# finmath/finmath-lib-cuda-extensions

Measured on AMD Instinct MI355X. Metric: Monte-Carlo path-ops/sec (fused RandomVariable stream), higher is better.
Workload: dtype f32

## Files before the change

finmath-lib-cuda-extensions_amd/host/hip_backend.hpp:

```cpp
#pragma once
#include <cstdlib>
#include <cstring>
#include <memory>
#include "lmm.hpp"

namespace fmhost {

class BrownianMotionFromMersenneRandomNumbersHip final : public BrownianMotion {
public:
    BrownianMotionFromMersenneRandomNumbersHip(TimeDiscretization td, int numberOfFactors, int64_t numberOfPaths, int seed, int64_t pathOffset = 0)
        : td_(std::move(td)), factors_(numberOfFactors), paths_(numberOfPaths), offset_(pathOffset), seed_(seed) {}
    RV getBrownianIncrement(int timeIndex, int factor) const override {
        std::call_once(generated_, [this] { generate(); });
        return inc_.at((size_t)timeIndex * factors_ + factor);
    }
    const TimeDiscretization& getTimeDiscretization() const override { return td_; }
    int getNumberOfFactors() const override { return factors_; }
    int64_t getNumberOfPaths() const override { return paths_; }
    int getSeed() const { return seed_; }
    RV getRandomVariableForConstant(double value) const override { return RandomVariableHip::of(-std::numeric_limits<double>::infinity(), value); }
private:
    void generate() const {
        const int steps = td_.getNumberOfTimeSteps();
        std::vector<double> dt((size_t)steps);
        for (int i = 0; i < steps; ++i) dt[(size_t)i] = td_.getTimeStep(i);
        std::vector<fmhip_vec> h((size_t)steps * factors_);
        check(fmhip_bm_generate_mersenne_device(seed_, steps, factors_, paths_, offset_, dt.data(), h.data()));
        inc_.reserve(h.size());
        for (int i = 0; i < steps; ++i)
            for (int f = 0; f < factors_; ++f)
                inc_.push_back(RandomVariableHip::of(td_.getTime(i + 1), DeviceVector(h[(size_t)i * factors_ + f]), paths_));
    }
    TimeDiscretization td_;
    int factors_;
    int64_t paths_, offset_;
    int seed_;
    mutable std::vector<RV> inc_;
    mutable std::once_flag generated_;
};

inline lmm::Backend makeHipBackend(const RandomVariableFactory* factory, const BrownianMotion* brownianMotion, int chunk = 0, int stepsPerLaunch = 0, int jacobianBatch = 0) {
    lmm::Backend be;
    be.factory = factory;
    be.brownianMotion = brownianMotion;
    if (!(std::getenv("FMHIP_LMM_FLUSH") && std::getenv("FMHIP_LMM_FLUSH")[0] == '0'))
        be.flush = [] { check(fmhip_flush()); };
    if (!(std::getenv("FMHIP_LMM_HOLD") && std::getenv("FMHIP_LMM_HOLD")[0] == '0'))
        be.hold = [](bool h) { check(fmhip_fusion_hold(h ? 1 : 0, nullptr)); };
    if (chunk > 0) be.chunk = chunk;
    if (stepsPerLaunch > 0) be.stepsPerLaunch = stepsPerLaunch;
    be.jacobianBatch = jacobianBatch > 0 ? jacobianBatch : 8;
    if (!(std::getenv("FMHIP_LMM_CLONE") && std::getenv("FMHIP_LMM_CLONE")[0] == '0')) {
        auto handleOf = [](const RV& x) {
            auto p = dynamic_cast<const RandomVariableHip*>(x.get());
            if (!p || p->isDeterministic()) throw std::runtime_error("graph replication over a value that is not a device vector");
            return p->deviceVector().handle();
        };
        be.clone = [handleOf](const std::vector<RV>& roots, const std::vector<RV>& leafFrom, const std::vector<std::vector<RV>>& leafTo,
                              const std::vector<std::vector<double>>* scalars) {
            const int nRoots = (int)roots.size(), nMap = (int)leafFrom.size(), nCopies = (int)leafTo.size();
            std::vector<fmhip_vec> r, lf, lt, out((size_t)nRoots * nCopies);
            for (const RV& x : roots) r.push_back(handleOf(x));
            for (const RV& x : leafFrom) lf.push_back(handleOf(x));
            for (const auto& row : leafTo) { if ((int)row.size() != nMap) throw std::runtime_error("graph replication: ragged operand map"); for (const RV& x : row) lt.push_back(handleOf(x)); }
            std::vector<double> sc;
            int nScalars = 0;
            if (scalars) { nScalars = (int)(*scalars)[0].size(); for (const auto& row : *scalars) { if ((int)row.size() != nScalars) throw std::runtime_error("graph replication: ragged scalar lists"); sc.insert(sc.end(), row.begin(), row.end()); } }
            check(fmhip_graph_clone(r.data(), nRoots, nCopies, lf.data(), lt.data(), nMap, scalars ? sc.data() : nullptr, nScalars, out.data()));
            std::vector<std::vector<RV>> copies((size_t)nCopies);
            for (int c = 0; c < nCopies; ++c)
                for (int k = 0; k < nRoots; ++k)
                    copies[(size_t)c].push_back(RandomVariableHip::of(roots[(size_t)k]->getFiltrationTime(), DeviceVector(out[(size_t)c * nRoots + k]), roots[(size_t)k]->size()));
            return copies;
        };
        be.recordedScalars = [handleOf](const std::vector<RV>& roots) {
            std::vector<fmhip_vec> r;
            for (const RV& x : roots) r.push_back(handleOf(x));
            int n = 0;
            check(fmhip_graph_scalars(r.data(), (int)r.size(), nullptr, 0, &n));
            std::vector<double> sc((size_t)n);
            check(fmhip_graph_scalars(r.data(), (int)r.size(), sc.data(), n, &n));
            return sc;
        };
    }
    if (!(std::getenv("FMHIP_LMM_DISCARD") && std::getenv("FMHIP_LMM_DISCARD")[0] == '0'))
        be.valuesNotNeeded = [](const std::vector<RV>& v) {
            std::vector<fmhip_vec> h;
            for (const RV& x : v) { auto p = dynamic_cast<const RandomVariableHip*>(x.get()); if (p && !p->isDeterministic()) h.push_back(p->deviceVector().handle()); }
            if (!h.empty()) check(fmhip_vec_give_up_values(h.data(), (int)h.size()));
        };
    be.launches = [] { fmhip_engine_stats_t s; check(fmhip_engine_stats(&s)); return (long long)s.kernel_launches; };
    be.averages = [](const std::vector<RV>& v) { return getAverages(v); };
    if (!(std::getenv("FMHIP_LMM_ASYNC") && std::getenv("FMHIP_LMM_ASYNC")[0] == '0'))
        be.expectationsRunPending = true;
    if (!(std::getenv("FMHIP_LMM_ASYNC") && std::getenv("FMHIP_LMM_ASYNC")[0] == '0'))
        be.averagesAsync = [](const std::vector<RV>& v) -> std::function<std::vector<double>()> {
            std::vector<fmhip_vec> h;
            int64_t n = 0;
            for (const RV& x : v) {
                auto p = dynamic_cast<const RandomVariableHip*>(x.get());
                if (!p || p->isDeterministic()) { const std::vector<double> now = getAverages(v); return [now] { return now; }; }
                h.push_back(p->deviceVector().handle()); n = p->size();
            }
            const int count = (int)h.size();
            fmhip_ticket ticket = 0;
            check(fmhip_reduce_moments_batch_begin(h.data(), count, nullptr, &ticket));
            struct Owner { fmhip_ticket t = 0; int count = 0; bool ended = false;
                           Owner() = default; Owner(const Owner&) = delete; Owner& operator=(const Owner&) = delete;
                           ~Owner() { if (!ended && t) { std::vector<fmhip_moments> drop((size_t)count); (void)fmhip_reduce_moments_batch_end(t, drop.data(), count); } } };
            auto owner = std::make_shared<Owner>();
            owner->t = ticket; owner->count = count;
            return [owner, count, n] {
                std::vector<fmhip_moments> m((size_t)count);
                owner->ended = true;
                check(fmhip_reduce_moments_batch_end(owner->t, m.data(), count));
                std::vector<double> out((size_t)count);
                for (int k = 0; k < count; ++k) out[(size_t)k] = m[(size_t)k].sum / (double)n;
                return out;
            };
        };
    return be;
}

}
```

finmath-lib-cuda-extensions_amd/host/lmm.hpp:

```cpp
#pragma once
#include <algorithm>
#include <chrono>
#include <cmath>
#include <cstdio>
#include <atomic>
#include <thread>
#include <cstdlib>
#include <functional>
#include <string>
#include <vector>

#include "random_variable.hpp"

namespace fmhost { namespace lmm {


inline const std::vector<double>& atmNormalVolatilities() {
    static const std::vector<double> v = {
        0.00151, 0.00169, 0.0021, 0.00248, 0.00291, 0.00329, 0.00365, 0.004, 0.00437, 0.00466, 0.00527, 0.00571,
        0.00604, 0.00625, 0.0016, 0.00174, 0.00217, 0.00264, 0.00314, 0.00355, 0.00398, 0.00433, 0.00469,
        0.00493, 0.00569, 0.00607, 0.00627, 0.00645, 0.00182, 0.00204, 0.00238, 0.00286, 0.00339, 0.00384,
        0.00424, 0.00456, 0.00488, 0.0052, 0.0059, 0.00623, 0.0064, 0.00654, 0.00205, 0.00235, 0.00272, 0.0032,
        0.00368, 0.00406, 0.00447, 0.00484, 0.00515, 0.00544, 0.00602, 0.00629, 0.0064, 0.00646, 0.00279,
        0.00319, 0.0036, 0.00396, 0.00436, 0.00469, 0.00503, 0.0053, 0.00557, 0.00582, 0.00616, 0.00628,
        0.00638, 0.00641, 0.00379, 0.00406, 0.00439, 0.00472, 0.00504, 0.00532, 0.0056, 0.00582, 0.00602,
        0.00617, 0.0063, 0.00636, 0.00638, 0.00639, 0.00471, 0.00489, 0.00511, 0.00539, 0.00563, 0.00583, 0.006,
        0.00618, 0.0063, 0.00644, 0.00641, 0.00638, 0.00635, 0.00634, 0.00544, 0.00557, 0.00572, 0.00591,
        0.00604, 0.00617, 0.0063, 0.00641, 0.00651, 0.00661, 0.00645, 0.00634, 0.00627, 0.00624, 0.00625,
        0.00632, 0.00638, 0.00644, 0.0065, 0.00655, 0.00661, 0.00667, 0.00672, 0.00673, 0.00634, 0.00614,
        0.00599, 0.00593, 0.00664, 0.00671, 0.00675, 0.00676, 0.00676, 0.00675, 0.00676, 0.00674, 0.00672,
        0.00669, 0.00616, 0.00586, 0.00569, 0.00558, 0.00647, 0.00651, 0.00651, 0.00651, 0.00652, 0.00649,
        0.00645, 0.0064, 0.00637, 0.00631, 0.00576, 0.00534, 0.00512, 0.00495, 0.00615, 0.0062, 0.00618,
        0.00613, 0.0061, 0.00607, 0.00602, 0.00596, 0.00591, 0.00586, 0.00536, 0.00491, 0.00469, 0.0045,
        0.00578, 0.00583, 0.00579, 0.00574, 0.00567, 0.00562, 0.00556, 0.00549, 0.00545, 0.00538, 0.00493,
        0.00453, 0.00435, 0.0042, 0.00542, 0.00547, 0.00539, 0.00532, 0.00522, 0.00516, 0.0051, 0.00504, 0.005,
        0.00495, 0.00454, 0.00418, 0.00404, 0.00394 };
    return v;
}
inline const std::vector<double>& atmExpiryYears() { static const std::vector<double> v = { 1.0 / 12, 0.25, 0.5, 1, 2, 3, 4, 5, 7, 10, 15, 20, 25, 30 }; return v; }
inline const std::vector<double>& atmTenorYears()  { static const std::vector<double> v = { 1, 2, 3, 4, 5, 6, 7, 8, 9, 10, 15, 20, 25, 30 }; return v; }

struct DiscountCurve {
    std::vector<double> t{ 0.0 }, logdf{ 0.0 };
    double df(double time) const {
        if (time <= 0.0) return 1.0;
        if (time >= t.back()) return std::exp(logdf.back());
        const size_t k = (size_t)(std::upper_bound(t.begin(), t.end(), time) - t.begin());
        const double w = (time - t[k - 1]) / (t[k] - t[k - 1]);
        return std::exp(logdf[k - 1] + w * (logdf[k] - logdf[k - 1]));
    }
    double forward(double fixing, double period) const { return (df(fixing) / df(fixing + period) - 1.0) / period; }
    static DiscountCurve bootstrap() {
        const double maturities[] = { 0.5, 1, 2, 3, 4, 5, 6, 7, 8, 9, 10, 11, 12, 15, 20, 25, 30, 35, 40, 45, 50 };
        const double rates[] = { -0.00216, -0.00208, -0.00222, -0.00216, -0.0019, -0.0014, -0.00072, 0.00011, 0.00103, 0.00196, 0.00285,
                                 0.00367, 0.0044, 0.00604, 0.00733, 0.00767, 0.00773, 0.00765, 0.00752, 0.007138, 0.007 };
        DiscountCurve c;
        for (int i = 0; i < 21; ++i) {
            const double M = maturities[i], r = rates[i];
            c.t.push_back(M); c.logdf.push_back(c.logdf.back());
            auto swapValue = [&](double ld) {
                c.logdf.back() = ld;
                double annuity = 0.0;
                if (M < 1.0) annuity = M * c.df(M);
                else for (double tp = 1.0; tp <= M + 1e-9; tp += 1.0) annuity += c.df(tp);
                return 1.0 - c.df(M) - r * annuity;
            };
            double lo = -3.0, hi = 1.0;
            for (int it = 0; it < 200; ++it) { const double mid = 0.5 * (lo + hi); if (swapValue(mid) > 0) lo = mid; else hi = mid; }
            c.logdf.back() = 0.5 * (lo + hi);
        }
        return c;
    }
};

struct Swaption {
    double exercise = 0; int numberOfPeriods = 0; double swapPeriodLength = 0.5;
    std::vector<double> swapTenor; double swaprate = 0, targetVolatility = 0, annuity = 0;
};

struct Market {
    DiscountCurve curve = DiscountCurve::bootstrap();
    double lastTime = 40.0, dt = 0.5;
    TimeDiscretization timeDiscretization{ 0.0, 80, 0.5 };
    std::vector<Swaption> swaptions;
    Market() {
        const auto& vols = atmNormalVolatilities();
        for (size_t e = 0; e < atmExpiryYears().size(); ++e)
            for (size_t k = 0; k < atmTenorYears().size(); ++k) {
                const double exercise = std::round(atmExpiryYears()[e] / 0.25) * 0.25, tenor = atmTenorYears()[k];
                if (exercise < 1.0) continue;
                if (exercise + tenor > lastTime + 1e-9) continue;
                Swaption s;
                s.exercise = exercise; s.numberOfPeriods = (int)std::lround(tenor / 0.5);
                for (int p = 0; p <= s.numberOfPeriods; ++p) s.swapTenor.push_back(exercise + p * 0.5);
                double floating = 0.0, annuity = 0.0;
                for (int p = 0; p < s.numberOfPeriods; ++p) {
                    const double d = curve.df(s.swapTenor[p + 1]);
                    floating += curve.forward(s.swapTenor[p], 0.5) * 0.5 * d; annuity += 0.5 * d;
                }
                s.swaprate = floating / annuity; s.annuity = annuity;
                s.targetVolatility = vols[e * atmTenorYears().size() + k];
                swaptions.push_back(std::move(s));
            }
    }
    int numberOfLibors() const { return timeDiscretization.getNumberOfTimeSteps(); }
};

struct VolatilityModel {
    std::vector<double> grid{ 0.0, 1.0, 2.0, 5.0, 10.0, 20.0, 30.0, 40.0 };
    std::vector<double> parameter = std::vector<double>(64, 0.50 / 100);
    int bin(double x) const { int k = 0; while (k < 7 && grid[(size_t)k] < x - 1e-12) ++k; return k; }
    int parameterIndex(double time, double maturity) const { return bin(time) * 8 + bin(maturity - time); }
    double volatility(double time, double maturity) const { return maturity <= time + 1e-12 ? 0.0 : parameter[(size_t)parameterIndex(time, maturity)]; }
    std::vector<int> activeParameters(const Market& m) const {
        std::vector<char> used(64, 0);
        const auto& td = m.timeDiscretization;
        for (int i = 0; i < td.getNumberOfTimeSteps(); ++i)
            for (int j = i + 1; j < m.numberOfLibors(); ++j) used[(size_t)parameterIndex(td.getTime(i), td.getTime(j))] = 1;
        std::vector<int> idx;
        for (int k = 0; k < 64; ++k) if (used[(size_t)k]) idx.push_back(k);
        return idx;
    }
};


struct Simulation {
    std::vector<std::vector<RV>> libor;
    std::vector<RV> numeraire;
};

struct Backend {
    const RandomVariableFactory* factory = nullptr;
    const BrownianMotion* brownianMotion = nullptr;
    std::function<void()> flush = [] {};
    std::function<void(bool)> hold = [](bool) {};
    std::function<long long()> launches = [] { return 0LL; };
    std::function<std::vector<double>(const std::vector<RV>&)> averages = [](const std::vector<RV>& v) {
        std::vector<double> a; for (const RV& x : v) a.push_back(x->getAverage()); return a; };
    std::function<std::function<std::vector<double>()>(const std::vector<RV>&)> averagesAsync;
    bool expectationsRunPending = false;
    std::function<void(const std::vector<RV>&)> valuesNotNeeded;
    int chunk = 7;
    int stepsPerLaunch = 4;
    std::function<std::vector<std::vector<RV>>(const std::vector<RV>& roots, const std::vector<RV>& leafFrom, const std::vector<std::vector<RV>>& leafTo,
                                               const std::vector<std::vector<double>>* scalars)> clone;
    std::function<std::vector<double>(const std::vector<RV>& roots)> recordedScalars;
    int jacobianBatch = 1;
    bool keepAllStates = false;
    int threads = 1;
};

inline std::vector<Simulation> simulateMany(const Market& m, const std::vector<const VolatilityModel*>& vols, const Backend& be, int lastTimeIndex,
                                            const std::vector<char>* keep = nullptr) {
    const auto& td = m.timeDiscretization;
    const int n = m.numberOfLibors();
    const double delta = m.dt;
    const size_t K = vols.size();
    std::vector<Simulation> sims(K);
    for (Simulation& sim : sims) {
        sim.libor.resize((size_t)lastTimeIndex + 1);
        sim.numeraire.resize((size_t)lastTimeIndex + 1);
        sim.libor[0].resize((size_t)n);
        for (int j = 0; j < n; ++j) sim.libor[0][(size_t)j] = be.factory->createRandomVariable(0.0, m.curve.forward(td.getTime(j), delta));
        sim.numeraire[0] = be.factory->createRandomVariable(0.0, 1.0);
    }
    std::vector<RV> factorSum(K);
    const int S = std::max(1, be.stepsPerLaunch);
    static int cloneChecks = 0;
    for (int i0 = 0; i0 < lastTimeIndex;) {
        int i1 = std::min(i0 + S, lastTimeIndex);
        static const bool endAtKept = std::getenv("FMHIP_LMM_GROUPS_END_AT_KEPT") && std::getenv("FMHIP_LMM_GROUPS_END_AT_KEPT")[0] == '1';
        if (keep && endAtKept) for (int s2 = i0 + 1; s2 < i1; ++s2) if ((*keep)[(size_t)s2]) { i1 = s2; break; }
        const bool cloning = K > 1 && S > 1 && keep && be.clone && i0 >= 2;
        const size_t Krec = cloning ? 1 : K;
        if (S > 1) be.hold(true);
        for (int i = i0; i < i1; ++i) {
            const double t = td.getTime(i), dt = td.getTimeStep(i);
            const RV dW = be.brownianMotion->getBrownianIncrement(i, 0);
            for (size_t k = 0; k < Krec; ++k) {
                auto& cur = sims[k].libor[(size_t)i];
                auto& nxt = sims[k].libor[(size_t)i + 1];
                nxt.resize((size_t)n);
                for (int j = 0; j <= i && j < n; ++j) nxt[(size_t)j] = cur[(size_t)j];
                factorSum[k] = nullptr;
            }
            for (int j0 = i + 1; j0 < n; j0 += be.chunk) {
                const int j1 = std::min(n, j0 + be.chunk);
                for (size_t k = 0; k < Krec; ++k) {
                    auto& cur = sims[k].libor[(size_t)i];
                    auto& nxt = sims[k].libor[(size_t)i + 1];
                    for (int j = j0; j < j1; ++j) {
                        const double lambda = vols[k]->volatility(t, td.getTime(j));
                        const RV& L = cur[(size_t)j];
                        const RV transform = be.factory->createRandomVariable(lambda * delta)->discount(L, delta);
                        factorSum[k] = factorSum[k] ? factorSum[k]->add(transform) : transform;
                        const RV drift = factorSum[k]->mult(lambda);
                        nxt[(size_t)j] = L->addProduct(drift, dt)->addProduct(dW, lambda);
                    }
                }
                if (S == 1 && j1 - j0 == be.chunk) be.flush();
            }
            for (size_t k = 0; k < Krec; ++k)
                sims[k].numeraire[(size_t)i + 1] = sims[k].numeraire[(size_t)i]->accrue(sims[k].libor[(size_t)i][(size_t)i], delta);
            for (size_t k = 0; k < Krec; ++k) factorSum[k] = nullptr;
        }
        if (cloning) {
            std::vector<RV> roots, leafFrom;
            for (int j = i0 + 1; j < n; ++j) roots.push_back(sims[0].libor[(size_t)i1][(size_t)j]);
            for (int i = i0; i < i1; ++i) roots.push_back(sims[0].numeraire[(size_t)i + 1]);
            for (int s2 = i0 + 1; s2 < i1; ++s2)
                if (!keep || (*keep)[(size_t)s2]) for (int j = s2; j < n; ++j) roots.push_back(sims[0].libor[(size_t)s2][(size_t)j]);
            for (int j = i0; j < n; ++j) leafFrom.push_back(sims[0].libor[(size_t)i0][(size_t)j]);
            leafFrom.push_back(sims[0].numeraire[(size_t)i0]);
            auto scalarsOf = [&](const VolatilityModel& vol) {
                std::vector<double> sc;
                for (int i = i0; i < i1; ++i) {
                    const double t = td.getTime(i), dt = td.getTimeStep(i);
                    for (int j = i + 1; j < n; ++j) {
                        const double lambda = vol.volatility(t, td.getTime(j));
                        sc.push_back(delta); sc.push_back(1.0); sc.push_back(lambda * delta); sc.push_back(lambda); sc.push_back(dt); sc.push_back(lambda);
                    }
                    sc.push_back(delta);
                }
                return sc;
            };
            if (cloneChecks < 64 && be.recordedScalars) {
                ++cloneChecks;
                if (be.recordedScalars(roots) != scalarsOf(*vols[0])) throw std::runtime_error("lmm: the scalar list of the replicated Euler steps does not match the recording");
            }
            std::vector<std::vector<RV>> leafTo(K - 1);
            std::vector<std::vector<double>> scalars(K - 1);
            for (size_t k = 1; k < K; ++k) {
                for (int j = i0; j < n; ++j) leafTo[k - 1].push_back(sims[k].libor[(size_t)i0][(size_t)j]);
                leafTo[k - 1].push_back(sims[k].numeraire[(size_t)i0]);
                scalars[k - 1] = scalarsOf(*vols[k]);
            }
            const std::vector<std::vector<RV>> copies = be.clone(roots, leafFrom, leafTo, &scalars);
            for (size_t k = 1; k < K; ++k) {
                auto& nxt = sims[k].libor[(size_t)i1];
                nxt.resize((size_t)n);
                for (int j = 0; j <= i0 && j < n; ++j) nxt[(size_t)j] = sims[k].libor[(size_t)i0][(size_t)j];
                size_t r = 0;
                for (int j = i0 + 1; j < n; ++j) nxt[(size_t)j] = copies[k - 1][r++];
                for (int i = i0; i < i1; ++i) sims[k].numeraire[(size_t)i + 1] = copies[k - 1][r++];
                for (int s2 = i0 + 1; s2 < i1; ++s2)
                    if (!keep || (*keep)[(size_t)s2]) { auto& mid = sims[k].libor[(size_t)s2]; mid.resize((size_t)n); for (int j = s2; j < n; ++j) mid[(size_t)j] = copies[k - 1][r++]; }
            }
        }
        if (keep)
            for (int i = i0; i < i1; ++i)
                if (!(*keep)[(size_t)i])
                    for (size_t k = 0; k < K; ++k) { sims[k].libor[(size_t)i].clear(); sims[k].libor[(size_t)i].shrink_to_fit(); }
        if (S > 1) be.hold(false);
        be.flush();
        i0 = i1;
    }
    return sims;
}

inline Simulation simulate(const Market& m, const VolatilityModel& vol, const Backend& be, int lastTimeIndex) {
    return std::move(simulateMany(m, { &vol }, be, lastTimeIndex)[0]);
}

inline RV swaptionValue(const Market& m, const Simulation& sim, const Swaption& s) {
    const auto& td = m.timeDiscretization;
    const int exerciseIndex = td.getTimeIndex(s.exercise);
    RV value;
    for (int p = s.numberOfPeriods - 1; p >= 0; --p) {
        const int j = td.getTimeIndex(s.swapTenor[(size_t)p]);
        const RV& libor = sim.libor[(size_t)exerciseIndex][(size_t)j];
        const RV payoff = libor->sub(s.swaprate)->mult(s.swapPeriodLength);
        value = (value ? value->add(payoff) : payoff)->discount(libor, s.swapPeriodLength);
    }
    return value->floor(0.0)->div(sim.numeraire[(size_t)exerciseIndex]);
}
inline double bachelierAtmImpliedVolatility(double optionValue, double optionMaturity, double annuity) {
    return optionValue * std::sqrt(2.0 * 3.14159265358979323846) / (annuity * std::sqrt(optionMaturity));
}

struct Valuation { std::vector<double> modelVolatility; double seconds_simulation = 0, seconds_valuation = 0; long long launches_simulation = 0, launches_valuation = 0; };

struct PendingValuations {
    std::vector<std::function<std::vector<double>()>> expectations;
    std::vector<Valuation> out;
};

inline std::vector<Valuation> evaluateManyFinish(const Market& m, PendingValuations& p) {
    for (size_t k = 0; k < p.out.size(); ++k) {
        const std::vector<double> optionValues = p.expectations[k]();
        for (size_t q = 0; q < m.swaptions.size(); ++q)
            p.out[k].modelVolatility.push_back(bachelierAtmImpliedVolatility(optionValues[q], m.swaptions[q].exercise, m.swaptions[q].annuity));
    }
    return std::move(p.out);
}

inline PendingValuations evaluateManyBegin(const Market& m, const std::vector<const VolatilityModel*>& vols, const Backend& be) {
    using clk = std::chrono::steady_clock;
    const size_t K = vols.size();
    PendingValuations pending;
    std::vector<Valuation>& out = pending.out;
    out.resize(K);
    int lastIndex = 0;
    for (const Swaption& s : m.swaptions) lastIndex = std::max(lastIndex, m.timeDiscretization.getTimeIndex(s.exercise));
    const auto t0 = clk::now();
    const long long l0 = be.launches();
    std::vector<char> keep((size_t)lastIndex + 1, 0);
    for (const Swaption& s : m.swaptions) keep[(size_t)m.timeDiscretization.getTimeIndex(s.exercise)] = 1;
    const std::vector<Simulation> sims = simulateMany(m, vols, be, lastIndex, be.keepAllStates ? nullptr : &keep);
    const auto t1 = clk::now();
    const long long l1 = be.launches();
    std::vector<std::vector<RV>> values(K);
    if (K > 1 && be.clone) {
        be.hold(true);
        values[0].reserve(m.swaptions.size());
        for (const Swaption& s : m.swaptions) values[0].push_back(swaptionValue(m, sims[0], s));
        std::vector<RV> leafFrom;
        std::vector<std::vector<RV>> leafTo(K - 1);
        for (int e = 0; e <= lastIndex; ++e) {
            if (!keep[(size_t)e]) continue;
            for (size_t k = 0; k < K; ++k) {
                std::vector<RV>& dst = k == 0 ? leafFrom : leafTo[k - 1];
                for (int j = e; j < m.numberOfLibors(); ++j) dst.push_back(sims[k].libor[(size_t)e][(size_t)j]);
                dst.push_back(sims[k].numeraire[(size_t)e]);
            }
        }
        const std::vector<std::vector<RV>> copies = be.clone(values[0], leafFrom, leafTo, nullptr);
        for (size_t k = 1; k < K; ++k) values[k] = copies[k - 1];
        be.hold(false);
        if (!(be.averagesAsync && be.expectationsRunPending)) be.flush();
    } else
    for (size_t k = 0; k < K; ++k) {
        be.hold(true);
        values[k].reserve(m.swaptions.size());
        for (const Swaption& s : m.swaptions) values[k].push_back(swaptionValue(m, sims[k], s));
        be.hold(false);
        if (!(be.averagesAsync && be.expectationsRunPending)) be.flush();
    }
    if (be.valuesNotNeeded) for (size_t k = 0; k < K; ++k) be.valuesNotNeeded(values[k]);
    for (size_t k = 0; k < K; ++k) {
        if (be.averagesAsync) pending.expectations.push_back(be.averagesAsync(values[k]));
        else { const std::vector<double> now = be.averages(values[k]); pending.expectations.push_back([now] { return now; }); }
    }
    const auto t2 = clk::now();
    for (size_t k = 0; k < K; ++k) {
        out[k].launches_simulation = (l1 - l0) / (long long)K; out[k].launches_valuation = (be.launches() - l1) / (long long)K;
        out[k].seconds_simulation = std::chrono::duration<double>(t1 - t0).count() / (double)K;
        out[k].seconds_valuation = std::chrono::duration<double>(t2 - t1).count() / (double)K;
    }
    return pending;
}

inline std::vector<Valuation> evaluateMany(const Market& m, const std::vector<const VolatilityModel*>& vols, const Backend& be) {
    PendingValuations p = evaluateManyBegin(m, vols, be);
    return evaluateManyFinish(m, p);
}

inline Valuation evaluate(const Market& m, const VolatilityModel& vol, const Backend& be) {
    return std::move(evaluateMany(m, { &vol }, be)[0]);
}


struct CalibrationResult {
    VolatilityModel model; int iterations = 0, evaluations = 0;
    double meanDeviation = 0, rmsDeviation = 0, initialRms = 0, seconds = 0, seconds_simulation = 0, seconds_valuation = 0;
    std::vector<double> modelVolatility;
};

inline bool solveSymmetric(std::vector<double> A, std::vector<double> b, int n, std::vector<double>& x) {
    for (int c = 0; c < n; ++c) {
        int piv = c;
        for (int r = c + 1; r < n; ++r) if (std::fabs(A[(size_t)r * n + c]) > std::fabs(A[(size_t)piv * n + c])) piv = r;
        if (std::fabs(A[(size_t)piv * n + c]) < 1e-300) return false;
        if (piv != c) { for (int k = 0; k < n; ++k) std::swap(A[(size_t)c * n + k], A[(size_t)piv * n + k]); std::swap(b[(size_t)c], b[(size_t)piv]); }
        for (int r = c + 1; r < n; ++r) {
            const double f = A[(size_t)r * n + c] / A[(size_t)c * n + c];
            for (int k = c; k < n; ++k) A[(size_t)r * n + k] -= f * A[(size_t)c * n + k];
            b[(size_t)r] -= f * b[(size_t)c];
        }
    }
    x.assign((size_t)n, 0.0);
    for (int r = n - 1; r >= 0; --r) { double s = b[(size_t)r]; for (int k = r + 1; k < n; ++k) s -= A[(size_t)r * n + k] * x[(size_t)k]; x[(size_t)r] = s / A[(size_t)r * n + r]; }
    return true;
}

inline CalibrationResult calibrate(const Market& m, const Backend& be, int maxIterations = 200, double accuracy = 1e-7,
                                   double lambda = 0.1, double parameterStep = 1e-4, bool verbose = false) {
    using clk = std::chrono::steady_clock;
    const auto start = clk::now();
    CalibrationResult res;
    VolatilityModel vol;
    const std::vector<int> active = vol.activeParameters(m);
    const int np = (int)active.size(), nr = (int)m.swaptions.size();
    auto residuals = [&](const VolatilityModel& v, std::vector<double>& r, std::vector<double>* modelVols) {
        const Valuation val = evaluate(m, v, be);
        res.evaluations++; res.seconds_simulation += val.seconds_simulation; res.seconds_valuation += val.seconds_valuation;
        r.resize((size_t)nr);
        for (int k = 0; k < nr; ++k) r[(size_t)k] = val.modelVolatility[(size_t)k] - m.swaptions[(size_t)k].targetVolatility;
        if (modelVols) *modelVols = val.modelVolatility;
    };
    auto sumsq = [](const std::vector<double>& r) { double s = 0; for (double x : r) s += x * x; return s; };
    std::vector<double> r, rTrial, modelVols;
    residuals(vol, r, &modelVols);
    double err = sumsq(r);
    res.initialRms = std::sqrt(err / nr);
    for (int it = 0; it < maxIterations; ++it) {
        std::vector<double> J((size_t)nr * np);
        struct InFlight { int a0 = 0, a1 = 0; std::vector<VolatilityModel> bumped; PendingValuations pending; bool valid = false; };
        auto collect = [&](InFlight& f) {
            if (!f.valid) return;
            const std::vector<Valuation> vals = evaluateManyFinish(m, f.pending);
            for (int a = f.a0; a < f.a1; ++a) {
                const Valuation& val = vals[(size_t)(a - f.a0)];
                res.evaluations++; res.seconds_simulation += val.seconds_simulation; res.seconds_valuation += val.seconds_valuation;
                for (int k = 0; k < nr; ++k) J[(size_t)k * np + a] = (val.modelVolatility[(size_t)k] - m.swaptions[(size_t)k].targetVolatility - r[(size_t)k]) / parameterStep;
            }
            f.valid = false;
        };
        if (be.threads > 1 && be.jacobianBatch <= 1) {
            const auto tj0 = clk::now();
            std::vector<Valuation> column((size_t)np);
            std::vector<std::string> failures((size_t)be.threads);
            std::atomic<int> next{ 0 };
            std::vector<std::thread> pool;
            for (int t = 0; t < be.threads; ++t)
                pool.emplace_back([&, t] {
                    try {
                        for (int a = next.fetch_add(1); a < np; a = next.fetch_add(1)) {
                            VolatilityModel bumped = vol;
                            bumped.parameter[(size_t)active[(size_t)a]] += parameterStep;
                            column[(size_t)a] = evaluate(m, bumped, be);
                        }
                    } catch (const std::exception& e) { failures[(size_t)t] = e.what(); }
                });
            for (std::thread& th : pool) th.join();
            if (std::getenv("FMHIP_LMM_TIMELINE")) std::fprintf(stderr, "[lmm timeline] iteration %d: %d columns on %d threads, %.3f … %.3f ms\n", it, np, be.threads, std::chrono::duration<double, std::milli>(tj0 - start).count(), std::chrono::duration<double, std::milli>(clk::now() - start).count());
            for (const std::string& f : failures) if (!f.empty()) throw std::runtime_error("a Jacobian column failed: " + f);
            for (int a = 0; a < np; ++a) {
                const Valuation& val = column[(size_t)a];
                res.evaluations++; res.seconds_simulation += val.seconds_simulation; res.seconds_valuation += val.seconds_valuation;
                for (int k = 0; k < nr; ++k) J[(size_t)k * np + a] = (val.modelVolatility[(size_t)k] - m.swaptions[(size_t)k].targetVolatility - r[(size_t)k]) / parameterStep;
            }
        } else {
        InFlight previous;
        for (int a0 = 0; a0 < np; a0 += std::max(1, be.jacobianBatch)) {
            const int a1 = std::min(np, a0 + std::max(1, be.jacobianBatch));
            InFlight current;
            current.a0 = a0; current.a1 = a1;
            current.bumped.assign((size_t)(a1 - a0), vol);
            std::vector<const VolatilityModel*> ptrs;
            for (int a = a0; a < a1; ++a) { current.bumped[(size_t)(a - a0)].parameter[(size_t)active[(size_t)a]] += parameterStep; ptrs.push_back(&current.bumped[(size_t)(a - a0)]); }
            static const bool timeline = std::getenv("FMHIP_LMM_TIMELINE") != nullptr;
            const auto tb0 = clk::now();
            try { current.pending = evaluateManyBegin(m, ptrs, be); current.valid = true; }
            catch (const std::exception& e) {
                if (ptrs.size() == 1 || std::string(e.what()).find("allocation") == std::string::npos) throw;
                if (verbose) std::fprintf(stderr, "  batch of %zu bumps does not fit (%s): evaluating them one at a time\n", ptrs.size(), e.what());
                be.flush();
                collect(previous);
                for (int a = a0; a < a1; ++a) {
                    const Valuation val = evaluate(m, current.bumped[(size_t)(a - a0)], be);
                    res.evaluations++; res.seconds_simulation += val.seconds_simulation; res.seconds_valuation += val.seconds_valuation;
                    for (int k = 0; k < nr; ++k) J[(size_t)k * np + a] = (val.modelVolatility[(size_t)k] - m.swaptions[(size_t)k].targetVolatility - r[(size_t)k]) / parameterStep;
                }
                continue;
            }
            const auto tb1 = clk::now();
            collect(previous);
            if (timeline) std::fprintf(stderr, "[lmm timeline] iteration %d batch from %d: begin %.3f … %.3f ms, previous collected at %.3f ms\n", it, a0,
                                       std::chrono::duration<double, std::milli>(tb0 - start).count(), std::chrono::duration<double, std::milli>(tb1 - start).count(),
                                       std::chrono::duration<double, std::milli>(clk::now() - start).count());
            previous = std::move(current);
        }
        collect(previous);
        }
        std::vector<double> JtJ((size_t)np * np, 0.0), Jtr((size_t)np, 0.0);
        for (int a = 0; a < np; ++a) {
            for (int b = 0; b < np; ++b) { double s = 0; for (int k = 0; k < nr; ++k) s += J[(size_t)k * np + a] * J[(size_t)k * np + b]; JtJ[(size_t)a * np + b] = s; }
            double s = 0; for (int k = 0; k < nr; ++k) s += J[(size_t)k * np + a] * r[(size_t)k]; Jtr[(size_t)a] = -s;
        }
        bool improved = false;
        for (int attempt = 0; attempt < 8 && !improved; ++attempt) {
            std::vector<double> A = JtJ, step;
            for (int a = 0; a < np; ++a) A[(size_t)a * np + a] += lambda * std::max(JtJ[(size_t)a * np + a], 1e-12);
            if (!solveSymmetric(A, Jtr, np, step)) { lambda *= 4; continue; }
            VolatilityModel v = vol;
            for (int a = 0; a < np; ++a) v.parameter[(size_t)active[(size_t)a]] += step[(size_t)a];
            std::vector<double> mv;
            const auto tt0 = clk::now();
            residuals(v, rTrial, &mv);
            static const bool timeline2 = std::getenv("FMHIP_LMM_TIMELINE") != nullptr;
            if (timeline2) std::fprintf(stderr, "[lmm timeline] iteration %d trial %d: %.3f … %.3f ms\n", it, attempt, std::chrono::duration<double, std::milli>(tt0 - start).count(),
                                        std::chrono::duration<double, std::milli>(clk::now() - start).count());
            const double e = sumsq(rTrial);
            if (e < err) { improved = true; const double rel = (err - e) / err; vol = v; r = rTrial; err = e; modelVols = mv; lambda = std::max(lambda / 3.0, 1e-9); if (rel < accuracy) it = maxIterations; }
            else lambda *= 4.0;
        }
        res.iterations++;
        if (verbose) std::fprintf(stderr, "  LM iteration %d: rms %.6e  lambda %.3g  evaluations %d\n", res.iterations, std::sqrt(err / nr), lambda, res.evaluations);
        if (!improved || std::sqrt(err / nr) < accuracy) break;
    }
    res.model = vol; res.modelVolatility = modelVols;
    double sum = 0; for (double x : r) sum += x;
    res.meanDeviation = sum / nr; res.rmsDeviation = std::sqrt(err / nr);
    res.seconds = std::chrono::duration<double>(clk::now() - start).count();
    return res;
}

}}
```

finmath-lib-cuda-extensions_amd/host/lmm_main_common.hpp:

```cpp
#pragma once
#include <vector>
#include <cstdlib>
#include <cstring>
#include <string>
#include "lmm.hpp"

namespace fmhost { namespace lmm {

struct Options {
    int64_t paths = 10000; int64_t seed = 31415; int maxIterations = 200; std::string mode = "calibrate"; bool verbose = false;
    int64_t pathOffset = 0; int evaluations = 1;
    int warmupEvaluations = 0;
    int world = 1, rank = 0; std::string ncclIdFile; long long ncclNonce = 0;
    std::vector<int> devices;
    int chunk = 0;
    int stepsPerLaunch = 0;
    int jacobianBatch = 0;
    std::string brownian = "philox";
    int threads = 1;
    double releaseLagMs = 0.0;
    long long releaseLagBytes = 0;
    bool finmathLike = false;
    bool profile = false;
};
inline Options parseOptions(int argc, char** argv) {
    Options o;
    for (int i = 1; i < argc; ++i) {
        const std::string a = argv[i];
        auto next = [&]() -> const char* { if (i + 1 >= argc) { std::fprintf(stderr, "missing value for %s\n", a.c_str()); std::exit(2); } return argv[++i]; };
        if (a == "--paths") o.paths = std::atoll(next());
        else if (a == "--seed") o.seed = std::atoll(next());
        else if (a == "--max-iterations") o.maxIterations = std::atoi(next());
        else if (a == "--mode") o.mode = next();
        else if (a == "--evaluations") o.evaluations = std::atoi(next());
        else if (a == "--warmup-evaluations") o.warmupEvaluations = std::atoi(next());
        else if (a == "--path-offset") o.pathOffset = std::atoll(next());
        else if (a == "--world") o.world = std::atoi(next());
        else if (a == "--devices") { std::string list = next(); size_t p0 = 0; while (p0 <= list.size()) { const size_t q = list.find(',', p0); o.devices.push_back(std::atoi(list.substr(p0, q == std::string::npos ? std::string::npos : q - p0).c_str())); if (q == std::string::npos) break; p0 = q + 1; } }
        else if (a == "--rank") o.rank = std::atoi(next());
        else if (a == "--nccl-id-file") o.ncclIdFile = next();
        else if (a == "--nccl-nonce") o.ncclNonce = std::atoll(next());
        else if (a == "--profile") o.profile = true;
        else if (a == "--finmath-like") o.finmathLike = true;
        else if (a == "--threads") o.threads = std::atoi(next());
        else if (a == "--release-lag") o.releaseLagMs = std::atof(next());
        else if (a == "--release-lag-bytes") o.releaseLagBytes = std::atoll(next());
        else if (a == "--brownian") o.brownian = next();
        else if (a == "--jacobian-batch") o.jacobianBatch = std::atoi(next());
        else if (a == "--chunk") o.chunk = std::atoi(next());
        else if (a == "--steps-per-launch") o.stepsPerLaunch = std::atoi(next());
        else if (a == "--verbose") o.verbose = true;
        else { std::fprintf(stderr, "unknown option %s\n", a.c_str()); std::exit(2); }
    }
    return o;
}

inline void runAndReport(const Options& o, const Backend& be, const char* backendName, const std::function<std::string()>& extraJson) {
    Market m;
    if (o.mode == "evaluate") {
        VolatilityModel vol;
        Valuation v;
        double sim = 0, val = 0;
        const int K = std::max(1, o.jacobianBatch);
        for (int k = 0; k < o.evaluations; k += K) {
            const int kk = std::min(K, o.evaluations - k);
            const std::vector<Valuation> vs = evaluateMany(m, std::vector<const VolatilityModel*>((size_t)kk, &vol), be);
            for (const Valuation& x : vs) { sim += x.seconds_simulation; val += x.seconds_valuation; }
            v = vs.back();
        }
        std::printf("{\"backend\": \"%s\", \"mode\": \"evaluate\", \"paths\": %lld, \"swaptions\": %zu, \"evaluations\": %d, "
                    "\"seconds_simulation_per_evaluation\": %.6f, \"seconds_valuation_per_evaluation\": %.6f, \"launches_simulation\": %lld, \"launches_valuation\": %lld%s, \"model_volatility\": [",
                    backendName, (long long)o.paths, m.swaptions.size(), o.evaluations, sim / o.evaluations, val / o.evaluations, v.launches_simulation, v.launches_valuation, extraJson().c_str());
        for (size_t k = 0; k < v.modelVolatility.size(); ++k) std::printf("%s%.17g", k ? ", " : "", v.modelVolatility[k]);
        std::printf("]}\n");
        return;
    }
    const CalibrationResult r = calibrate(m, be, o.maxIterations, 1e-7, 0.1, 1e-4, o.verbose);
    std::printf("{\"backend\": \"%s\", \"mode\": \"calibrate\", \"paths\": %lld, \"swaptions\": %zu, \"active_parameters\": %zu, "
                "\"iterations\": %d, \"evaluations\": %d, \"seconds\": %.4f, \"seconds_simulation\": %.4f, \"seconds_valuation\": %.4f, "
                "\"initial_rms\": %.6e, \"rms_deviation\": %.6e, \"mean_deviation\": %.6e%s, \"parameters\": [",
                backendName, (long long)o.paths, m.swaptions.size(), VolatilityModel().activeParameters(m).size(), r.iterations, r.evaluations,
                r.seconds, r.seconds_simulation, r.seconds_valuation, r.initialRms, r.rmsDeviation, r.meanDeviation, extraJson().c_str());
    for (size_t k = 0; k < r.model.parameter.size(); ++k) std::printf("%s%.17g", k ? ", " : "", r.model.parameter[k]);
    std::printf("]}\n");
}

}}
```

Baseline: 4207 billion.

## Deduplicate identical bumped simulations and add memory-aware Jacobian batch planning

In a Jacobian batch, scenarios whose state and per-step scalars are identical are grouped into classes. Only one representative per class records or clones the Euler steps and the swaption valuations, and the other members share its results. The shared initial LIBOR and numeraire constants are built once for all scenarios. An opt-in 'auto' Jacobian batch size sizes batches from free device memory. The goal is to skip redundant simulation and valuation work for parameter bumps that do not change early time steps, at the cost of extra host-side pointer and scalar comparisons.

New measurement: 3911 billion. -7.0%, worse.

```diff
diff --git a/finmath-lib-cuda-extensions_amd/host/hip_backend.hpp b/finmath-lib-cuda-extensions_amd/host/hip_backend.hpp
--- a/finmath-lib-cuda-extensions_amd/host/hip_backend.hpp
+++ b/finmath-lib-cuda-extensions_amd/host/hip_backend.hpp
@@ -49,7 +49,12 @@
         be.hold = [](bool h) { check(fmhip_fusion_hold(h ? 1 : 0, nullptr)); };
     if (chunk > 0) be.chunk = chunk;
     if (stepsPerLaunch > 0) be.stepsPerLaunch = stepsPerLaunch;
-    be.jacobianBatch = jacobianBatch > 0 ? jacobianBatch : 8;
+    be.jacobianBatch = jacobianBatch > 0 ? jacobianBatch : jacobianBatch < 0 ? 0 : 8;
+    be.freeDeviceBytes = [] {
+        fmhip_pool_stats_t s; check(fmhip_pool_stats(&s));
+        int shards = 1; check(fmhip_device_count(&shards));
+        return ((long long)s.device_bytes_free + (long long)s.bytes_cached) / std::max(1, shards);
+    };
     if (!(std::getenv("FMHIP_LMM_CLONE") && std::getenv("FMHIP_LMM_CLONE")[0] == '0')) {
         auto handleOf = [](const RV& x) {
             auto p = dynamic_cast<const RandomVariableHip*>(x.get());
diff --git a/finmath-lib-cuda-extensions_amd/host/lmm.hpp b/finmath-lib-cuda-extensions_amd/host/lmm.hpp
--- a/finmath-lib-cuda-extensions_amd/host/lmm.hpp
+++ b/finmath-lib-cuda-extensions_amd/host/lmm.hpp
@@ -6,6 +6,7 @@
 #include <atomic>
 #include <thread>
 #include <cstdlib>
+#include <cstring>
 #include <functional>
 #include <string>
 #include <vector>
@@ -146,23 +147,84 @@
                                                const std::vector<std::vector<double>>* scalars)> clone;
     std::function<std::vector<double>(const std::vector<RV>& roots)> recordedScalars;
     int jacobianBatch = 1;
+    std::function<long long()> freeDeviceBytes;
     bool keepAllStates = false;
     int threads = 1;
 };
 
+
+inline long long bytesPerParameterSet(const Market& m, long long paths) {
+    const int n = m.numberOfLibors();
+    std::vector<char> kept((size_t)n + 1, 0);
+    for (const Swaption& s : m.swaptions) kept[(size_t)m.timeDiscretization.getTimeIndex(s.exercise)] = 1;
+    long long vectors = 2LL * n;
+    for (int e = 0; e <= n; ++e) if (kept[(size_t)e]) vectors += n - e + 1;
+    return 4LL * paths * vectors;
+}
+
+constexpr double jacobianMemoryFraction = 0.7;
+
+inline std::vector<int> jacobianBatchPlanWithin(int np, long long bytesPerSet, double budgetBytes) {
+    if (np <= 0) return {};
+    const long long fit = bytesPerSet > 0 ? (long long)std::floor(std::max(0.0, budgetBytes) / (double)bytesPerSet) : np;
+    const int most = (int)std::min<long long>(np, std::max<long long>(1, fit));
+    const int batches = (np + most - 1) / most;
+    std::vector<int> sizes((size_t)batches, np / batches);
+    for (int b = 0; b < np % batches; ++b) sizes[(size_t)b] += 1;
+    return sizes;
+}
+inline std::vector<int> jacobianBatchPlan(int np, long long bytesPerSet, long long freeBytes) {
+    return jacobianBatchPlanWithin(np, bytesPerSet, jacobianMemoryFraction * (double)std::max(0LL, freeBytes));
+}
+
+inline std::vector<int> jacobianBatches(int np, const Backend& be, long long bytesPerSet) {
+    int fixed = be.jacobianBatch;
+    if (fixed <= 0 && !be.freeDeviceBytes) fixed = 8;
+    if (fixed > 0) {
+        std::vector<int> sizes;
+        for (int a0 = 0; a0 < np; a0 += fixed) sizes.push_back(std::min(fixed, np - a0));
+        return sizes;
+    }
+    if (const char* e = std::getenv("FMHIP_LMM_JACOBIAN_BUDGET_BYTES")) {
+        return jacobianBatchPlanWithin(np, bytesPerSet, (double)std::atoll(e));
+    }
+    return jacobianBatchPlan(np, bytesPerSet, be.freeDeviceBytes());
+}
+
+inline std::vector<double> stepGroupScalars(const Market& m, const VolatilityModel& vol, int i0, int i1) {
+    const auto& td = m.timeDiscretization;
+    const int n = m.numberOfLibors();
+    const double delta = m.dt;
+    std::vector<double> sc;
+    sc.reserve((size_t)(i1 - i0) * (6 * (size_t)n + 1));
+    for (int i = i0; i < i1; ++i) {
+        const double t = td.getTime(i), dt = td.getTimeStep(i);
+        for (int j = i + 1; j < n; ++j) {
+            const double lambda = vol.volatility(t, td.getTime(j));
+            sc.push_back(delta); sc.push_back(1.0); sc.push_back(lambda * delta); sc.push_back(lambda); sc.push_back(dt); sc.push_back(lambda);
+        }
+        sc.push_back(delta);
+    }
+    return sc;
+}
+
 inline std::vector<Simulation> simulateMany(const Market& m, const std::vector<const VolatilityModel*>& vols, const Backend& be, int lastTimeIndex,
-                                            const std::vector<char>* keep = nullptr) {
+                                            const std::vector<char>* keep = nullptr, std::vector<std::vector<size_t>>* classesOut = nullptr) {
     const auto& td = m.timeDiscretization;
     const int n = m.numberOfLibors();
     const double delta = m.dt;
     const size_t K = vols.size();
     std::vector<Simulation> sims(K);
-    for (Simulation& sim : sims) {
-        sim.libor.resize((size_t)lastTimeIndex + 1);
-        sim.numeraire.resize((size_t)lastTimeIndex + 1);
-        sim.libor[0].resize((size_t)n);
-        for (int j = 0; j < n; ++j) sim.libor[0][(size_t)j] = be.factory->createRandomVariable(0.0, m.curve.forward(td.getTime(j), delta));
-        sim.numeraire[0] = be.factory->createRandomVariable(0.0, 1.0);
+    {
+        std::vector<RV> libor0((size_t)n);
+        for (int j = 0; j < n; ++j) libor0[(size_t)j] = be.factory->createRandomVariable(0.0, m.curve.forward(td.getTime(j), delta));
+        const RV numeraire0 = be.factory->createRandomVariable(0.0, 1.0);
+        for (Simulation& sim : sims) {
+            sim.libor.resize((size_t)lastTimeIndex + 1);
+            sim.numeraire.resize((size_t)lastTimeIndex + 1);
+            sim.libor[0] = libor0;
+            sim.numeraire[0] = numeraire0;
+        }
     }
     std::vector<RV> factorSum(K);
     const int S = std::max(1, be.stepsPerLaunch);
@@ -171,13 +233,31 @@
         int i1 = std::min(i0 + S, lastTimeIndex);
         static const bool endAtKept = std::getenv("FMHIP_LMM_GROUPS_END_AT_KEPT") && std::getenv("FMHIP_LMM_GROUPS_END_AT_KEPT")[0] == '1';
         if (keep && endAtKept) for (int s2 = i0 + 1; s2 < i1; ++s2) if ((*keep)[(size_t)s2]) { i1 = s2; break; }
+        std::vector<size_t> representativeOf(K, 0), representatives{ 0 };
+        std::vector<std::vector<double>> scalarsOf(K);
+        if (K > 1) {
+            auto sameState = [&](size_t a, size_t b) {
+                if (sims[a].numeraire[(size_t)i0].get() != sims[b].numeraire[(size_t)i0].get()) return false;
+                for (int j = i0; j < n; ++j) if (sims[a].libor[(size_t)i0][(size_t)j].get() != sims[b].libor[(size_t)i0][(size_t)j].get()) return false;
+                return true;
+            };
+            for (size_t k = 0; k < K; ++k) scalarsOf[k] = stepGroupScalars(m, *vols[k], i0, i1);
+            for (size_t k = 1; k < K; ++k) {
+                size_t found = k;
+                for (size_t r : representatives)
+                    if (sameState(r, k) && std::memcmp(scalarsOf[r].data(), scalarsOf[k].data(), scalarsOf[k].size() * sizeof(double)) == 0) { found = r; break; }
+                representativeOf[k] = found;
+                if (found == k) representatives.push_back(k);
+            }
+        }
+        if (classesOut) classesOut->push_back(representativeOf);
         const bool cloning = K > 1 && S > 1 && keep && be.clone && i0 >= 2;
-        const size_t Krec = cloning ? 1 : K;
+        const std::vector<size_t> recorded = cloning ? std::vector<size_t>{ 0 } : representatives;
         if (S > 1) be.hold(true);
         for (int i = i0; i < i1; ++i) {
             const double t = td.getTime(i), dt = td.getTimeStep(i);
             const RV dW = be.brownianMotion->getBrownianIncrement(i, 0);
-            for (size_t k = 0; k < Krec; ++k) {
+            for (size_t k : recorded) {
                 auto& cur = sims[k].libor[(size_t)i];
                 auto& nxt = sims[k].libor[(size_t)i + 1];
                 nxt.resize((size_t)n);
@@ -186,7 +266,7 @@
             }
             for (int j0 = i + 1; j0 < n; j0 += be.chunk) {
                 const int j1 = std::min(n, j0 + be.chunk);
-                for (size_t k = 0; k < Krec; ++k) {
+                for (size_t k : recorded) {
                     auto& cur = sims[k].libor[(size_t)i];
                     auto& nxt = sims[k].libor[(size_t)i + 1];
                     for (int j = j0; j < j1; ++j) {
@@ -200,9 +280,9 @@
                 }
                 if (S == 1 && j1 - j0 == be.chunk) be.flush();
             }
-            for (size_t k = 0; k < Krec; ++k)
+            for (size_t k : recorded)
                 sims[k].numeraire[(size_t)i + 1] = sims[k].numeraire[(size_t)i]->accrue(sims[k].libor[(size_t)i][(size_t)i], delta);
-            for (size_t k = 0; k < Krec; ++k) factorSum[k] = nullptr;
+            for (size_t k : recorded) factorSum[k] = nullptr;
         }
         if (cloning) {
             std::vector<RV> roots, leafFrom;
@@ -212,40 +292,38 @@
                 if (!keep || (*keep)[(size_t)s2]) for (int j = s2; j < n; ++j) roots.push_back(sims[0].libor[(size_t)s2][(size_t)j]);
             for (int j = i0; j < n; ++j) leafFrom.push_back(sims[0].libor[(size_t)i0][(size_t)j]);
             leafFrom.push_back(sims[0].numeraire[(size_t)i0]);
-            auto scalarsOf = [&](const VolatilityModel& vol) {
-                std::vector<double> sc;
-                for (int i = i0; i < i1; ++i) {
-                    const double t = td.getTime(i), dt = td.getTimeStep(i);
-                    for (int j = i + 1; j < n; ++j) {
-                        const double lambda = vol.volatility(t, td.getTime(j));
-                        sc.push_back(delta); sc.push_back(1.0); sc.push_back(lambda * delta); sc.push_back(lambda); sc.push_back(dt); sc.push_back(lambda);
-                    }
-                    sc.push_back(delta);
-                }
-                return sc;
-            };
             if (cloneChecks < 64 && be.recordedScalars) {
                 ++cloneChecks;
-                if (be.recordedScalars(roots) != scalarsOf(*vols[0])) throw std::runtime_error("lmm: the scalar list of the replicated Euler steps does not match the recording");
-            }
-            std::vector<std::vector<RV>> leafTo(K - 1);
-            std::vector<std::vector<double>> scalars(K - 1);
-            for (size_t k = 1; k < K; ++k) {
-                for (int j = i0; j < n; ++j) leafTo[k - 1].push_back(sims[k].libor[(size_t)i0][(size_t)j]);
-                leafTo[k - 1].push_back(sims[k].numeraire[(size_t)i0]);
-                scalars[k - 1] = scalarsOf(*vols[k]);
-            }
-            const std::vector<std::vector<RV>> copies = be.clone(roots, leafFrom, leafTo, &scalars);
-            for (size_t k = 1; k < K; ++k) {
-                auto& nxt = sims[k].libor[(size_t)i1];
-                nxt.resize((size_t)n);
-                for (int j = 0; j <= i0 && j < n; ++j) nxt[(size_t)j] = sims[k].libor[(size_t)i0][(size_t)j];
-                size_t r = 0;
-                for (int j = i0 + 1; j < n; ++j) nxt[(size_t)j] = copies[k - 1][r++];
-                for (int i = i0; i < i1; ++i) sims[k].numeraire[(size_t)i + 1] = copies[k - 1][r++];
-                for (int s2 = i0 + 1; s2 < i1; ++s2)
-                    if (!keep || (*keep)[(size_t)s2]) { auto& mid = sims[k].libor[(size_t)s2]; mid.resize((size_t)n); for (int j = s2; j < n; ++j) mid[(size_t)j] = copies[k - 1][r++]; }
-            }
+                if (be.recordedScalars(roots) != scalarsOf[0]) throw std::runtime_error("lmm: the scalar list of the replicated Euler steps does not match the recording");
+            }
+            const size_t copiesWanted = representatives.size() - 1;
+            if (copiesWanted > 0) {
+                std::vector<std::vector<RV>> leafTo(copiesWanted);
+                std::vector<std::vector<double>> scalars(copiesWanted);
+                for (size_t c = 0; c < copiesWanted; ++c) {
+                    const size_t k = representatives[c + 1];
+                    for (int j = i0; j < n; ++j) leafTo[c].push_back(sims[k].libor[(size_t)i0][(size_t)j]);
+                    leafTo[c].push_back(sims[k].numeraire[(size_t)i0]);
+                    scalars[c] = std::move(scalarsOf[k]);
+                }
+                const std::vector<std::vector<RV>> copies = be.clone(roots, leafFrom, leafTo, &scalars);
+                for (size_t c = 0; c < copiesWanted; ++c) {
+                    const size_t k = representatives[c + 1];
+                    auto& nxt = sims[k].libor[(size_t)i1];
+                    nxt.resize((size_t)n);
+                    for (int j = 0; j <= i0 && j < n; ++j) nxt[(size_t)j] = sims[k].libor[(size_t)i0][(size_t)j];
+                    size_t r = 0;
+                    for (int j = i0 + 1; j < n; ++j) nxt[(size_t)j] = copies[c][r++];
+                    for (int i = i0; i < i1; ++i) sims[k].numeraire[(size_t)i + 1] = copies[c][r++];
+                    for (int s2 = i0 + 1; s2 < i1; ++s2)
+                        if (!keep || (*keep)[(size_t)s2]) { auto& mid = sims[k].libor[(size_t)s2]; mid.resize((size_t)n); for (int j = s2; j < n; ++j) mid[(size_t)j] = copies[c][r++]; }
+                }
+            }
+        }
+        for (size_t k = 1; k < K; ++k) {
+            const size_t r = representativeOf[k];
+            if (r == k) continue;
+            for (int i = i0; i < i1; ++i) { sims[k].libor[(size_t)i + 1] = sims[r].libor[(size_t)i + 1]; sims[k].numeraire[(size_t)i + 1] = sims[r].numeraire[(size_t)i + 1]; }
         }
         if (keep)
             for (int i = i0; i < i1; ++i)
@@ -309,34 +387,65 @@
     const std::vector<Simulation> sims = simulateMany(m, vols, be, lastIndex, be.keepAllStates ? nullptr : &keep);
     const auto t1 = clk::now();
     const long long l1 = be.launches();
-    std::vector<std::vector<RV>> values(K);
+    const int n = m.numberOfLibors();
+    std::vector<int> exerciseIndexOf(m.swaptions.size());
+    for (size_t q = 0; q < m.swaptions.size(); ++q) exerciseIndexOf[q] = m.timeDiscretization.getTimeIndex(m.swaptions[q].exercise);
+    std::vector<std::vector<size_t>> representativeAt((size_t)lastIndex + 1);
+    for (int e = 0; e <= lastIndex; ++e) {
+        if (!keep[(size_t)e]) continue;
+        std::vector<size_t>& rep = representativeAt[(size_t)e];
+        rep.assign(K, 0);
+        std::vector<size_t> distinct{ 0 };
+        for (size_t k = 1; k < K; ++k) {
+            size_t found = k;
+            for (size_t r : distinct) {
+                bool same = sims[r].numeraire[(size_t)e].get() == sims[k].numeraire[(size_t)e].get();
+                for (int j = e; same && j < n; ++j) same = sims[r].libor[(size_t)e][(size_t)j].get() == sims[k].libor[(size_t)e][(size_t)j].get();
+                if (same) { found = r; break; }
+            }
+            rep[k] = found;
+            if (found == k) distinct.push_back(k);
+        }
+    }
+    auto ownsValue = [&](size_t k, size_t q) { return representativeAt[(size_t)exerciseIndexOf[q]][k] == k; };
+    std::vector<std::vector<RV>> values(K, std::vector<RV>(m.swaptions.size()));
     if (K > 1 && be.clone) {
         be.hold(true);
-        values[0].reserve(m.swaptions.size());
-        for (const Swaption& s : m.swaptions) values[0].push_back(swaptionValue(m, sims[0], s));
-        std::vector<RV> leafFrom;
-        std::vector<std::vector<RV>> leafTo(K - 1);
+        for (size_t q = 0; q < m.swaptions.size(); ++q) values[0][q] = swaptionValue(m, sims[0], m.swaptions[q]);
         for (int e = 0; e <= lastIndex; ++e) {
             if (!keep[(size_t)e]) continue;
-            for (size_t k = 0; k < K; ++k) {
-                std::vector<RV>& dst = k == 0 ? leafFrom : leafTo[k - 1];
-                for (int j = e; j < m.numberOfLibors(); ++j) dst.push_back(sims[k].libor[(size_t)e][(size_t)j]);
+            std::vector<size_t> owners, products;
+            for (size_t k = 1; k < K; ++k) if (representativeAt[(size_t)e][k] == k) owners.push_back(k);
+            for (size_t q = 0; q < m.swaptions.size(); ++q) if (exerciseIndexOf[q] == e) products.push_back(q);
+            if (owners.empty() || products.empty()) continue;
+            std::vector<RV> roots, leafFrom;
+            std::vector<std::vector<RV>> leafTo(owners.size());
+            for (size_t q : products) roots.push_back(values[0][q]);
+            for (size_t c = 0; c <= owners.size(); ++c) {
+                const size_t k = c == 0 ? 0 : owners[c - 1];
+                std::vector<RV>& dst = c == 0 ? leafFrom : leafTo[c - 1];
+                for (int j = e; j < n; ++j) dst.push_back(sims[k].libor[(size_t)e][(size_t)j]);
                 dst.push_back(sims[k].numeraire[(size_t)e]);
             }
-        }
-        const std::vector<std::vector<RV>> copies = be.clone(values[0], leafFrom, leafTo, nullptr);
-        for (size_t k = 1; k < K; ++k) values[k] = copies[k - 1];
+            const std::vector<std::vector<RV>> copies = be.clone(roots, leafFrom, leafTo, nullptr);
+            for (size_t c = 0; c < owners.size(); ++c)
+                for (size_t i = 0; i < products.size(); ++i) values[owners[c]][products[i]] = copies[c][i];
+        }
         be.hold(false);
         if (!(be.averagesAsync && be.expectationsRunPending)) be.flush();
     } else
     for (size_t k = 0; k < K; ++k) {
         be.hold(true);
-        values[k].reserve(m.swaptions.size());
-        for (const Swaption& s : m.swaptions) values[k].push_back(swaptionValue(m, sims[k], s));
+        for (size_t q = 0; q < m.swaptions.size(); ++q) if (ownsValue(k, q)) values[k][q] = swaptionValue(m, sims[k], m.swaptions[q]);
         be.hold(false);
         if (!(be.averagesAsync && be.expectationsRunPending)) be.flush();
     }
-    if (be.valuesNotNeeded) for (size_t k = 0; k < K; ++k) be.valuesNotNeeded(values[k]);
+    for (size_t k = 1; k < K; ++k)
+        for (size_t q = 0; q < m.swaptions.size(); ++q) if (!ownsValue(k, q)) values[k][q] = values[representativeAt[(size_t)exerciseIndexOf[q]][k]][q];
+    if (be.valuesNotNeeded) {
+        std::vector<RV> own;
+        for (size_t k = 0; k < K; ++k) { own.clear(); for (size_t q = 0; q < m.swaptions.size(); ++q) if (ownsValue(k, q)) own.push_back(values[k][q]); if (!own.empty()) be.valuesNotNeeded(own); }
+    }
     for (size_t k = 0; k < K; ++k) {
         if (be.averagesAsync) pending.expectations.push_back(be.averagesAsync(values[k]));
         else { const std::vector<double> now = be.averages(values[k]); pending.expectations.push_back([now] { return now; }); }
@@ -364,6 +473,8 @@
     VolatilityModel model; int iterations = 0, evaluations = 0;
     double meanDeviation = 0, rmsDeviation = 0, initialRms = 0, seconds = 0, seconds_simulation = 0, seconds_valuation = 0;
     std::vector<double> modelVolatility;
+    std::vector<int> jacobianBatches;
+    long long bytesPerParameterSet = 0;
 };
 
 inline bool solveSymmetric(std::vector<double> A, std::vector<double> b, int n, std::vector<double>& x) {
@@ -391,6 +502,8 @@
     VolatilityModel vol;
     const std::vector<int> active = vol.activeParameters(m);
     const int np = (int)active.size(), nr = (int)m.swaptions.size();
+    const long long bytesPerSet = bytesPerParameterSet(m, be.brownianMotion ? (long long)be.brownianMotion->getNumberOfPaths() : 0);
+    res.bytesPerParameterSet = bytesPerSet;
     auto residuals = [&](const VolatilityModel& v, std::vector<double>& r, std::vector<double>* modelVols) {
         const Valuation val = evaluate(m, v, be);
         res.evaluations++; res.seconds_simulation += val.seconds_simulation; res.seconds_valuation += val.seconds_valuation;
@@ -442,8 +555,11 @@
             }
         } else {
         InFlight previous;
-        for (int a0 = 0; a0 < np; a0 += std::max(1, be.jacobianBatch)) {
-            const int a1 = std::min(np, a0 + std::max(1, be.jacobianBatch));
+        const std::vector<int> batches = jacobianBatches(np, be, bytesPerSet);
+        if (it == 0) res.jacobianBatches = batches;
+        int a0 = 0, a1 = 0;
+        for (size_t batch = 0; batch < batches.size(); ++batch, a0 = a1) {
+            a1 = a0 + batches[batch];
             InFlight current;
             current.a0 = a0; current.a1 = a1;
             current.bumped.assign((size_t)(a1 - a0), vol);
diff --git a/finmath-lib-cuda-extensions_amd/host/lmm_main_common.hpp b/finmath-lib-cuda-extensions_amd/host/lmm_main_common.hpp
--- a/finmath-lib-cuda-extensions_amd/host/lmm_main_common.hpp
+++ b/finmath-lib-cuda-extensions_amd/host/lmm_main_common.hpp
@@ -46,7 +46,7 @@
         else if (a == "--release-lag") o.releaseLagMs = std::atof(next());
         else if (a == "--release-lag-bytes") o.releaseLagBytes = std::atoll(next());
         else if (a == "--brownian") o.brownian = next();
-        else if (a == "--jacobian-batch") o.jacobianBatch = std::atoi(next());
+        else if (a == "--jacobian-batch") { const std::string v = next(); o.jacobianBatch = v == "auto" ? -1 : std::atoi(v.c_str()); }
         else if (a == "--chunk") o.chunk = std::atoi(next());
         else if (a == "--steps-per-launch") o.stepsPerLaunch = std::atoi(next());
         else if (a == "--verbose") o.verbose = true;
@@ -78,9 +78,11 @@
     const CalibrationResult r = calibrate(m, be, o.maxIterations, 1e-7, 0.1, 1e-4, o.verbose);
     std::printf("{\"backend\": \"%s\", \"mode\": \"calibrate\", \"paths\": %lld, \"swaptions\": %zu, \"active_parameters\": %zu, "
                 "\"iterations\": %d, \"evaluations\": %d, \"seconds\": %.4f, \"seconds_simulation\": %.4f, \"seconds_valuation\": %.4f, "
-                "\"initial_rms\": %.6e, \"rms_deviation\": %.6e, \"mean_deviation\": %.6e%s, \"parameters\": [",
+                "\"initial_rms\": %.6e, \"rms_deviation\": %.6e, \"mean_deviation\": %.6e, \"bytes_per_parameter_set\": %lld, \"jacobian_batches\": [",
                 backendName, (long long)o.paths, m.swaptions.size(), VolatilityModel().activeParameters(m).size(), r.iterations, r.evaluations,
-                r.seconds, r.seconds_simulation, r.seconds_valuation, r.initialRms, r.rmsDeviation, r.meanDeviation, extraJson().c_str());
+                r.seconds, r.seconds_simulation, r.seconds_valuation, r.initialRms, r.rmsDeviation, r.meanDeviation, r.bytesPerParameterSet);
+    for (size_t k = 0; k < r.jacobianBatches.size(); ++k) std::printf("%s%d", k ? ", " : "", r.jacobianBatches[k]);
+    std::printf("]%s, \"parameters\": [", extraJson().c_str());
     for (size_t k = 0; k < r.model.parameter.size(); ++k) std::printf("%s%.17g", k ? ", " : "", r.model.parameter[k]);
     std::printf("]}\n");
 }
```
